# metaverse3d2022/Nerf-Cuda

Measured on AMD Instinct MI355X. Metric: megasamples/s (march samples composited into a ray = the reference's per-ray sample count), Lego-like NeRF render @1920x1080, higher is better.
Workload: dtype f16

## Files before the change

nerf-cuda_amd/csrc/nrf_device.h:

```cpp
#pragma once

#include <hip/hip_runtime.h>
#include <stdint.h>

#include "../../include/nerfhip.h"

namespace nrf {

typedef _Float16 half_t;
typedef _Float16 half2_t __attribute__((ext_vector_type(2)));
typedef _Float16 half4_t __attribute__((ext_vector_type(4)));
typedef _Float16 half8_t __attribute__((ext_vector_type(8)));
typedef float float2_t __attribute__((ext_vector_type(2)));
typedef float float4_t __attribute__((ext_vector_type(4)));

enum : uint32_t {
  LV_DENSE = 0,
  LV_HASH_POW2 = 1,
  LV_GENERIC = 2,
  LV_ADD_POW2 = 3
};

struct LevelParams {
  float scale;
// ... 287 lines not shown
  uint32_t log2H;
  float halfH;
  int log2_bound;
};

__device__ __forceinline__ MarchConst march_const(const DevModel& M, float dt_gamma) {
  MarchConst c;
  c.bound = M.bound;
  c.rbound = M.rbound;
  c.dt_gamma = dt_gamma;
  c.dt_min = 2 * 1.7320508075688772f / 1024;
  c.dt_max = 2 * M.bound / (float)M.H;
  c.H = M.H;
  c.C = M.cascade;
  c.HH = M.H * M.H;
  c.HHH = M.H * M.H * M.H;
  c.Hf = (float)M.H;
  c.Hm1 = (float)(M.H - 1);
  c.coarse_shift = M.coarse_shift;
  c.Hc = M.H >> M.coarse_shift;
  c.log2H = 31u - (uint32_t)__builtin_clz(M.H | 1u);
  c.halfH = 0.5f * (float)M.H;
  {
    int e;
    (void)frexpf(M.bound, &e);
    c.log2_bound = e - 1;
  }
  return c;
}

__device__ __forceinline__ float pcg32_first_float(uint64_t initstate, uint64_t initseq) {
  const uint64_t MULT = 0x5851f42d4c957f2dULL;
  const uint64_t inc = (initseq << 1u) | 1u;
  uint64_t state = inc;
  state += initstate;
  state = state * MULT + inc;
  const uint32_t xorshifted = (uint32_t)(((state >> 18u) ^ state) >> 27u);
  const uint32_t rot = (uint32_t)(state >> 59u);
  const uint32_t r = (xorshifted >> rot) | (xorshifted << ((~rot + 1u) & 31u));
  return __builtin_bit_cast(float, (r >> 9) | 0x3f800000u) - 1.0f;
}

enum : int { MARCH_FOUND = 0, MARCH_EXHAUSTED = 1, MARCH_OUT_OF_BUDGET = 2 };

__device__ __forceinline__ float clamp3(float x, float lo, float hi) { return __builtin_amdgcn_fmed3f(x, lo, hi); }

enum : int { MARCH_GENERIC = 0, MARCH_UNIT = 1, MARCH_POW2 = 2 };
template <bool COARSE, int MODE>
__device__ __forceinline__ int march_next(const MarchConst& c, const uint32_t* __restrict__ occ, const uint32_t* coarse,
                                          const float* ctab, float ox, float oy, float oz, float dx, float dy, float dz,
                                          float rdx, float rdy, float rdz, int sx, int sy, int sz, float far, float t_skip,
                                          int& budget, float& t, float& x, float& y, float& z, float& dt_out) {
  while (t < far) {
    if (budget <= 0) return MARCH_OUT_OF_BUDGET;
    --budget;
#ifdef NRF_DIAG_EXTRA_MARCH
#pragma unroll
    for (int e = 0; e < NRF_DIAG_EXTRA_MARCH; ++e) {
      float sink;
      asm volatile("v_mul_f32 %0, %1, %2" : "=v"(sink) : "v"(t), "v"(dx));
    }
#endif
#ifdef NRF_DIAG_FF_UPPER
    if (t < t_skip) {
      do {
        t += clamp3(t * c.dt_gamma, c.dt_min, c.dt_max);
      } while (t < t_skip && t < far);
      continue;
    }
#endif
    x = clamp3(ox + t * dx, -c.bound, c.bound);
    y = clamp3(oy + t * dy, -c.bound, c.bound);
    z = clamp3(oz + t * dz, -c.bound, c.bound);
    constexpr bool UNIT = MODE == MARCH_UNIT, POW2 = MODE == MARCH_POW2;
    int level = 0;
    int nx, ny, nz;
    if (UNIT) {
      nx = (int)clamp3(__builtin_fmaf(x, c.halfH, c.halfH), 0.0f, c.Hm1);
      ny = (int)clamp3(__builtin_fmaf(y, c.halfH, c.halfH), 0.0f, c.Hm1);
      nz = (int)clamp3(__builtin_fmaf(z, c.halfH, c.halfH), 0.0f, c.Hm1);
    } else if (POW2) {
      const float mx = fmaxf(fabsf(x), fmaxf(fabsf(y), fabsf(z)));
      int exponent;
      (void)frexpf(mx, &exponent);
      level = min(max(exponent, 0), (int)c.C - 1);
      const float scale = ldexpf(c.halfH, -min(level, c.log2_bound));
      nx = (int)clamp3(__builtin_fmaf(x, scale, c.halfH), 0.0f, c.Hm1);
      ny = (int)clamp3(__builtin_fmaf(y, scale, c.halfH), 0.0f, c.Hm1);
      nz = (int)clamp3(__builtin_fmaf(z, scale, c.halfH), 0.0f, c.Hm1);
    } else {
      float mip_bound = fminf(1.0f, c.bound), mip_rbound;
      if (c.C > 1) {
        const float mx = fmaxf(fabsf(x), fmaxf(fabsf(y), fabsf(z)));
        int exponent;
        (void)frexpf(mx, &exponent);
        level = (int)fminf((float)c.C - 1, fmaxf(0.0f, (float)exponent));
        mip_bound = fminf(ldexpf(1.0f, level), c.bound);
      }
      mip_rbound = (mip_bound == c.bound) ? c.rbound : ldexpf(1.0f, -level);
      nx = (int)clamp3((0.5f * (x * mip_rbound + 1)) * c.Hf, 0.0f, c.Hm1);
      ny = (int)clamp3((0.5f * (y * mip_rbound + 1)) * c.Hf, 0.0f, c.Hm1);
      nz = (int)clamp3((0.5f * (z * mip_rbound + 1)) * c.Hf, 0.0f, c.Hm1);
    }
    const uint32_t cell = (UNIT || POW2) ? ((((((uint32_t)level << c.log2H) | (uint32_t)nx) << c.log2H) | (uint32_t)ny) << c.log2H) | (uint32_t)nz
                                         : (uint32_t)level * c.HHH + (uint32_t)nx * c.HH + (uint32_t)ny * c.H + (uint32_t)nz;
    const float* tab = UNIT ? ctab : ctab + (uint32_t)level * (c.H + 1);
    const float bx = tab[nx + sx], by = tab[ny + sy], bz = tab[nz + sz];
    bool occupied = false;
    if (!(t < t_skip)) {
      if (COARSE) {
        const uint32_t lc = c.log2H - 2u;
        const uint32_t cc = (UNIT || POW2) ? (((((((uint32_t)level << lc) | ((uint32_t)nx >> 2)) << lc) | ((uint32_t)ny >> 2)) << lc) | ((uint32_t)nz >> 2))
                                           : ((uint32_t)level * c.Hc + ((uint32_t)nx >> 2)) * c.Hc * c.Hc + ((uint32_t)ny >> 2) * c.Hc + ((uint32_t)nz >> 2);
        const bool coarse_occ = (coarse[cc >> 5] >> (cc & 31u)) & 1u;
        if (coarse_occ) occupied = (occ[cell >> 5] >> (cell & 31u)) & 1u;
      } else {
        occupied = (occ[cell >> 5] >> (cell & 31u)) & 1u;
      }
    }
    if (occupied) {
      dt_out = clamp3(t * c.dt_gamma, c.dt_min, c.dt_max);
      return MARCH_FOUND;
    }
    const float tx = (bx - x) * rdx;
    const float ty = (by - y) * rdy;
    const float tz = (bz - z) * rdz;
    const float tt = t + fmaxf(0.0f, fminf(tx, fminf(ty, tz)));
    do {
      t += clamp3(t * c.dt_gamma, c.dt_min, c.dt_max);
    } while (t < tt);
  }
  return MARCH_EXHAUSTED;
}

#ifndef NRF_MARCH_FF
#define NRF_MARCH_FF 1
#endif
__device__ __forceinline__ float barrier_before(const float* ctab, int H, float mb, float mag, float o, float d, float rd, float t_skip) {
  const float NONE = -3.402823466e+38f;
  if (!(d < 0.0f) || !(rd > -3.0e38f)) return NONE;
  const float xs = o + t_skip * d;
  const float v = clamp3(ceilf((xs / mb + 1.0f) * (0.5f * (float)(H - 1))), 0.0f, (float)H);
  int n = (int)v;
  if (n > H - 1) return NONE;
  const float eps = 4.0e-6f * mag * (1.0f + fabsf(rd));
  float e = (ctab[n] - o) * rd + eps;
  if (!(e <= t_skip)) {
    if (++n > H - 1) return NONE;
    e = (ctab[n] - o) * rd + eps;
  }
  return e <= t_skip ? e : NONE;
}

__device__ __forceinline__ float fast_forward_to_barrier(const MarchConst& c, const float* ctab, float mb, const float o[3], const float d[3],
                                                         float rdx, float rdy, float rdz, float t, float t_skip, float far) {
  const float mag = t_skip + c.bound + 2.0f;
  const float tb = fminf(fmaxf(barrier_before(ctab, (int)c.H, mb, mag, o[0], d[0], rdx, t_skip),
                               fmaxf(barrier_before(ctab, (int)c.H, mb, mag, o[1], d[1], rdy, t_skip),
                                     barrier_before(ctab, (int)c.H, mb, mag, o[2], d[2], rdz, t_skip))), far);
  while (t < tb) t += clamp3(t * c.dt_gamma, c.dt_min, c.dt_max);
  return t;
}

__device__ __forceinline__ bool cube_interval(float s, const float o[3], const float rd[3], float& t_in, float& t_out) {
  bool ok = true;
  t_in = -3.402823466e+38f;
  t_out = 3.402823466e+38f;
#pragma unroll
  for (int a = 0; a < 3; ++a) {
    const float u = (-s - o[a]) * rd[a], v = (s - o[a]) * rd[a];
    ok = ok && (u == u) && (v == v);
    t_in = fmaxf(t_in, fminf(u, v));
    t_out = fminf(t_out, fmaxf(u, v));
  }
  return ok;
}

__device__ __forceinline__ float fast_forward_to_barrier_pow2(const MarchConst& c, const float* ctab, const float o[3], const float d[3],
                                                              float rdx, float rdy, float rdz, float t, float t_skip, float far) {
  const float NONE = -3.402823466e+38f;
  const float rd[3] = {rdx, rdy, rdz};
  const int C = (int)c.C, H = (int)c.H;
  const float mag = t_skip + c.bound + 2.0f;
  const float pad = 1.0e-4f * mag;
  const float slab0 = 2.0f / (float)H;
  float t_hi = t_skip, best = NONE;
  for (int it = 0; it <= C && !(best > NONE) && t_hi > t; ++it) {
    const float qx = clamp3(o[0] + t_hi * d[0], -c.bound, c.bound), qy = clamp3(o[1] + t_hi * d[1], -c.bound, c.bound),
                qz = clamp3(o[2] + t_hi * d[2], -c.bound, c.bound);
    int ex;
    (void)frexpf(fmaxf(fabsf(qx), fmaxf(fabsf(qy), fabsf(qz))), &ex);
    const int L = min(max(ex, 0), C - 1);
    const float mb = fminf(ldexpf(1.0f, L), c.bound);
    const float* tab = ctab + (uint32_t)L * (uint32_t)(H + 1);
    const float slab_next = slab0 * fminf(ldexpf(1.0f, L + 1), c.bound);
    const bool has_in = L >= 1, has_out = L <= C - 2;
    float ai = 0.f, bi = 0.f, ao = 0.f, bo = 0.f;
    const bool ok_in = has_in ? cube_interval(ldexpf(1.0f, L - 1) + pad, o, rd, ai, bi) : true;
    const bool ok_out = has_out ? cube_interval(ldexpf(1.0f, L) - pad, o, rd, ao, bo) : true;
#pragma unroll
    for (int a = 0; a < 3; ++a) {
      if (!(d[a] < 0.0f) || !(rd[a] > -3.0e38f)) continue;
      const float ard = fabsf(rd[a]);
      const float eps = 4.0e-6f * mag * (1.0f + ard);
      const float xs = o[a] + t_hi * d[a];
      int n = (int)clamp3(ceilf((xs / mb + 1.0f) * (0.5f * (float)(H - 1))), 0.0f, (float)H);
      if (n > H - 1) continue;
      float T = (tab[n] - o[a]) * rd[a], e = T + eps;
      if (!(e <= t_hi)) {
        if (++n > H - 1) continue;
        T = (tab[n] - o[a]) * rd[a];
        e = T + eps;
      }
      if (!(e <= t_hi)) continue;
      const float w_lo = T - slab_next * ard - eps;
      bool ok = ok_in && ok_out;
      if (has_out) ok = ok && ao <= w_lo && e <= bo;
      if (has_in) ok = ok && (ai > bi || e <= ai || w_lo >= bi);
      for (int Lp = L + 2; Lp <= C - 1 && ok; ++Lp) {
        float a2, b2;
        ok = cube_interval(ldexpf(1.0f, Lp - 1) - pad, o, rd, a2, b2);
        ok = ok && a2 <= T - slab0 * fminf(ldexpf(1.0f, Lp), c.bound) * ard - eps && e <= b2;
      }
      if (ok) best = fmaxf(best, e);
    }
    if (best > NONE) break;
    float nxt = NONE;
    const float lim = t_hi - 1.0e-6f * mag;
    if (has_in && ok_in) {
      if (ai < lim) nxt = fmaxf(nxt, ai);
      if (bi < lim) nxt = fmaxf(nxt, bi);
    }
    if (has_out && ok_out) {
      if (ao < lim) nxt = fmaxf(nxt, ao);
      if (bo < lim) nxt = fmaxf(nxt, bo);
    }
    t_hi = nxt - 4.0f * pad;
  }
  const float tb = fminf(best, far);
  while (t < tb) t += clamp3(t * c.dt_gamma, c.dt_min, c.dt_max);
  return t;
}

__device__ __forceinline__ half2_t weight_times_entry(float w, uint32_t entry) {
  float lo, hi;
  const float neg_zero = -0.0f;
  asm("v_fma_mix_f32 %0, %1, %2, %3 op_sel_hi:[0,1,0]" : "=v"(lo) : "v"(w), "v"(entry), "v"(neg_zero));
  asm("v_fma_mix_f32 %0, %1, %2, %3 op_sel:[0,1,0] op_sel_hi:[0,1,0]" : "=v"(hi) : "v"(w), "v"(entry), "v"(neg_zero));
  half2_t p;
  p.x = (half_t)lo;
  p.y = (half_t)hi;
  return p;
}

template <int UNI = 0, int SH = 2>
__device__ __forceinline__ void level_offsets(const LevelParams L, float px, float py, float pz, uint32_t (&off)[8], float (&frac)[3]) {
  float fx = px * L.scale; fx = fx + 0.5f;
  float fy = py * L.scale; fy = fy + 0.5f;
  float fz = pz * L.scale; fz = fz + 0.5f;
  const uint32_t gx = (uint32_t)(int)fx, gy = (uint32_t)(int)fy, gz = (uint32_t)(int)fz;
  frac[0] = __builtin_amdgcn_fractf(fx);
  frac[1] = __builtin_amdgcn_fractf(fy);
  frac[2] = __builtin_amdgcn_fractf(fz);

  const uint32_t level_off = L.off_b;
  {
    const bool hashed = UNI == 2 || (UNI == 0 && L.mode == LV_HASH_POW2);
    const uint32_t my = UNI == 2 ? (2654435761u << SH) : L.my_b;
    const uint32_t mz = UNI == 2 ? (805459861u << SH) : L.mz_b;
    const uint32_t mask = UNI == 1 ? 0xffffffffu : L.mask_b;
    const uint32_t ax0 = (gx << SH) + (hashed ? 0u : level_off);
    const uint32_t ax[2] = {ax0, ax0 + (1u << SH)};
    const uint32_t ay0 = gy * my, az0 = gz * mz;
    const uint32_t ay[2] = {ay0, ay0 + my};
    const uint32_t az[2] = {az0, az0 + mz};
    if (UNI == 2) {
      const uint32_t am[2] = {(ax[0] & mask) | level_off, (ax[1] & mask) | level_off};
      uint32_t bd[4];
#pragma unroll
      for (int q = 0; q < 4; ++q) bd[q] = (ay[q & 1] ^ az[q >> 1]) & mask;
#pragma unroll
      for (int c = 0; c < 8; ++c) off[c] = am[c & 1] ^ bd[c >> 1];
    } else if (UNI == 1) {
#pragma unroll
      for (int c = 0; c < 8; ++c) off[c] = ax[c & 1] + ay[(c >> 1) & 1] + az[(c >> 2) & 1];
    } else {
      const uint32_t axr[2] = {gx << SH, (gx << SH) + (1u << SH)};
      const uint32_t am[2] = {(axr[0] & mask) | level_off, (axr[1] & mask) | level_off};
#pragma unroll
      for (int q = 0; q < 4; ++q) {
        const uint32_t b = ay[q & 1], d = az[q >> 1];
        const uint32_t bd_x = (b ^ d) & mask, bd_s = b + d;
#pragma unroll
        for (int e = 0; e < 2; ++e) off[2 * q + e] = hashed ? (am[e] ^ bd_x) : (((axr[e] + bd_s) & mask) + level_off);
      }
    }
  }
}

template <int UNI = 0>
__device__ __forceinline__ void level_gather(const uint32_t* __restrict__ grid, uint32_t grid_bytes, const LevelParams L, float px,
                                             float py, float pz, uint32_t (&v)[8], float (&frac)[3]) {
  uint32_t off[8];
  level_offsets<UNI, 2>(L, px, py, pz, off, frac);
  const __amdgpu_buffer_rsrc_t rsrc = __builtin_amdgcn_make_buffer_rsrc(const_cast<uint32_t*>(grid), 0, grid_bytes, 0x00020000);
#ifdef NRF_DIAG_HASH_PAIRS
  if (UNI == 2) {
    typedef uint32_t u32x2 __attribute__((ext_vector_type(2)));
#pragma unroll
    for (int q = 0; q < 4; ++q) {
      const u32x2 w = __builtin_amdgcn_raw_buffer_load_b64(rsrc, off[2 * q] & ~4u, 0, 0);
      v[2 * q] = w.x;
      v[2 * q + 1] = w.y;
    }
    return;
  }
#endif
#pragma unroll
  for (int c = 0; c < 8; ++c) v[c] = __builtin_amdgcn_raw_buffer_load_b32(rsrc, off[c], 0, 0);
}

__device__ __forceinline__ void level_gather_quad(const uint32_t* __restrict__ grid, uint32_t grid_bytes, const LevelParams L, float px,
                                                  float py, float pz, uint32_t (&v)[8], float (&frac)[3]) {
  float fx = px * L.scale; fx = fx + 0.5f;
  float fy = py * L.scale; fy = fy + 0.5f;
  float fz = pz * L.scale; fz = fz + 0.5f;
  const uint32_t gx = (uint32_t)(int)fx, gy = (uint32_t)(int)fy, gz = (uint32_t)(int)fz;
  frac[0] = __builtin_amdgcn_fractf(fx);
  frac[1] = __builtin_amdgcn_fractf(fy);
  frac[2] = __builtin_amdgcn_fractf(fz);
  const uint32_t row = __umul24(gy, L.q_my_b) + L.q_off_b;
  const uint32_t slab = __umul24(gz, L.q_mz_b) + row;
  const uint32_t off0 = (gx << 4) + slab;
  const uint32_t off1 = off0 + L.q_mz_b;
  const __amdgpu_buffer_rsrc_t rsrc = __builtin_amdgcn_make_buffer_rsrc(const_cast<uint32_t*>(grid), 0, grid_bytes, 0x00020000);
  typedef uint32_t u32x4 __attribute__((ext_vector_type(4)));
  const u32x4 a = __builtin_amdgcn_raw_buffer_load_b128(rsrc, off0, 0, 0);
  const u32x4 b = __builtin_amdgcn_raw_buffer_load_b128(rsrc, off1, 0, 0);
  v[0] = a.x; v[1] = a.y; v[2] = a.z; v[3] = a.w;
  v[4] = b.x; v[5] = b.y; v[6] = b.z; v[7] = b.w;
}

__device__ __forceinline__ void level_gather_quad_far(const uint32_t* __restrict__ grid, const LevelParams L, float px, float py, float pz,
                                                      uint32_t (&v)[8], float (&frac)[3]) {
  float fx = px * L.scale; fx = fx + 0.5f;
  float fy = py * L.scale; fy = fy + 0.5f;
  float fz = pz * L.scale; fz = fz + 0.5f;
  uint32_t gx = (uint32_t)(int)fx, gy = (uint32_t)(int)fy, gz = (uint32_t)(int)fz;
  frac[0] = __builtin_amdgcn_fractf(fx);
  frac[1] = __builtin_amdgcn_fractf(fy);
  frac[2] = __builtin_amdgcn_fractf(fz);
  gx = gx < L.q_max ? gx : L.q_max;
  gy = gy < L.q_max ? gy : L.q_max;
  gz = gz < L.q_max ? gz : L.q_max;
  const uint32_t row = __umul24(gy, L.q_my_b) + L.q_off_b;
  const uint32_t cell = __umul24(gz, L.q_mz_b) + row + gx;
  const uint4* q = reinterpret_cast<const uint4*>(grid) + cell;
  const uint4 a = q[0];
  const uint4 b = q[L.q_mz_b];
  v[0] = a.x; v[1] = a.y; v[2] = a.z; v[3] = a.w;
  v[4] = b.x; v[5] = b.y; v[6] = b.z; v[7] = b.w;
}

template <bool FAST = false>
__device__ __forceinline__ uint32_t level_interp(const uint32_t (&v)[8], const float (&frac)[3]) {
  const float wx[2] = {1 - frac[0], frac[0]};
  const float wy[2] = {1 - frac[1], frac[1]};
  const float wz[2] = {1 - frac[2], frac[2]};
  if constexpr (FAST) {
    uint32_t a = 0u;
#pragma unroll
    for (int c = 0; c < 8; ++c) {
      const float w = (wx[c & 1] * wy[(c >> 1) & 1]) * wz[(c >> 2) & 1];
      asm("v_fma_mixlo_f16 %0, %1, %2, %0 op_sel_hi:[0,1,1]" : "+v"(a) : "v"(w), "v"(v[c]));
      asm("v_fma_mixhi_f16 %0, %1, %2, %0 op_sel:[0,1,1] op_sel_hi:[0,1,1]" : "+v"(a) : "v"(w), "v"(v[c]));
    }
    return a;
  }
  half2_t acc = {(half_t)0.0f, (half_t)0.0f};
#ifdef NRF_DIAG_DROP_INTERP_CVT
  float diag_acc_lo = 0.f, diag_acc_hi = 0.f;
#endif
#pragma unroll
  for (int c = 0; c < 8; ++c) {
    const float w = (wx[c & 1] * wy[(c >> 1) & 1]) * wz[(c >> 2) & 1];
#ifdef NRF_DIAG_DROP_INTERP_CVT
    {
      float lo, hi;
      const float neg_zero = -0.0f;
      asm("v_fma_mix_f32 %0, %1, %2, %3 op_sel_hi:[0,1,0]" : "=v"(lo) : "v"(w), "v"(v[c]), "v"(neg_zero));
      asm("v_fma_mix_f32 %0, %1, %2, %3 op_sel:[0,1,0] op_sel_hi:[0,1,0]" : "=v"(hi) : "v"(w), "v"(v[c]), "v"(neg_zero));
      diag_acc_lo += lo;
      diag_acc_hi += hi;
    }
// ... 482 lines not shown
```

nerf-cuda_amd/csrc/nrf_render.h:

```cpp

#pragma once
#include <cstddef>
#include <cstdlib>

#include "nrf_device.h"
#include "nrf_generic.h"
#include "nrf_launch.h"

namespace nrf {

#ifndef NRF_SLOTS
#define NRF_SLOTS 64
#endif
constexpr int SLOTS = NRF_SLOTS;
struct WaveLds {
  union {
    float4 pos[SLOTS];
    float4 out[SLOTS];
  };
  float2 aux[SLOTS];
  uint32_t dirf[64][8];
};
static_assert(sizeof(WaveLds) == 2048 + 24 * SLOTS, "WaveLds layout");

// ... 988 lines not shown
        }
        if (!(c_in < c_out)) continue;
        float t_last, t_first;
        const uint32_t* dl_g = M.occ_dilated + (size_t)k * M.dilated_level_words;
        const uint32_t* dl_l = dil_lds + (size_t)k * M.dilated_level_words;
        const bool vis = use_dil_lds ? coarse_visibility(dl_l, Hc, mb, o, d, rdx, rdy, rdz, c_in, c_out, t_first, t_last)
                                     : coarse_visibility(dl_g, Hc, mb, o, d, rdx, rdy, rdz, c_in, c_out, t_first, t_last);
        if (vis) {
          any = true;
          first = fminf(first, t_first);
          last = fmaxf(last, t_last);
        }
      }
      alive = any;
      if (last < far_m) far_m = last;
      if (any) t_skip = first;
#if NRF_MARCH_FF
      if (any && P.march_ff != 0) {
        const float* tab = COARSE_LDS ? ctab_lds : M.cell_bound;
        if (MARCH == MARCH_UNIT) t = fast_forward_to_barrier(mc, tab, 1.0f, o, d, rdx, rdy, rdz, t, t_skip, far_m);
        else if (MARCH == MARCH_POW2 || mc.C > 1) t = fast_forward_to_barrier_pow2(mc, tab, o, d, rdx, rdy, rdz, t, t_skip, far_m);
        else t = fast_forward_to_barrier(mc, tab, fminf(1.0f, mc.bound), o, d, rdx, rdy, rdz, t, t_skip, far_m);
      }
#endif
    }
    if (RAYS != RAYS_DENSITY && alive) {
      float u0 = 0.5f * d[0]; u0 = u0 + 0.5f;
      float u1 = 0.5f * d[1]; u1 = u1 + 0.5f;
      float u2 = 0.5f * d[2]; u2 = u2 + 0.5f;
      if constexpr (GEN) {
        lm.gen.rayd[3 * lane] = u0;
        lm.gen.rayd[3 * lane + 1] = u1;
        lm.gen.rayd[3 * lane + 2] = u2;
      } else {
        half_t e[16];
        encode_dir16(M, u0, u1, u2, e);
#pragma unroll
        for (int j = 0; j < 8; ++j) {
          half2_t h;
          h.x = e[2 * j];
          h.y = e[2 * j + 1];
          W->dirf[lane][j] = h2_bits(h);
        }
        if constexpr (NET == NET_WIDE) {
          lm.gen.rayd[3 * lane] = u0;
          lm.gen.rayd[3 * lane + 1] = u1;
          lm.gen.rayd[3 * lane + 2] = u2;
        }
      }
    }
    if (__syncthreads_or(alive ? 1 : 0) != 0) {
      if constexpr (!GEN) {
        stage_fragments<NET>(M, wl);
        __syncthreads();
      }
    }
  }
  if (!valid_tile) return;
  NRF_STAMP(t_setup_done);
  TileAcc acc;
  TileStats ts;
  const uint32_t pix_idx = P.tile_major ? (uint32_t)k_local * 64u + (uint32_t)lane : (uint32_t)py * (uint32_t)P.W + (uint32_t)px;
  tile_rounds<NET, COARSE_LDS, MARCH, false, false, PERTURB, RAYS>(M, P, mc, lm, coarse_lds, ctab_lds, lane, o, d, rdx, rdy, rdz, sx, sy, sz,
                                                                   far_m, t_skip, t, tc, alive, acc, ts, 0, nullptr, pix_idx, 0.f, 0.f, nullptr,
                                                                   view);
  const unsigned n_samples = ts.n_samples, n_rounds = ts.n_rounds, n_tile_slots = ts.n_tile_slots;
  const unsigned n_composited = ts.n_composited;
#ifdef NRF_PHASE_TIMING
  const unsigned long long c_march = ts.c_march, c_net = ts.c_net, c_comp = ts.c_comp;
  const unsigned n_lane_trips = ts.n_lane_trips, n_wave_iters = ts.n_wave_iters;
#endif

  {
    const uint32_t rn = (uint32_t)py * (uint32_t)P.W + (uint32_t)px;
    float dn;
    const float4 c = finish_pixel<RAYS != RAYS_NONE>(P, acc, near, far, view, rn, in_img && rn < P.rays_per_view, dn);
    store_pixel(P, rgba, depth, k_local, lane, px, py, in_img, c, dn);
  }
  counters += (blockIdx.x % COUNTER_SLOTS) * 16;
  if (lane == 0 && n_rounds != 0) {
    atomicAdd(&counters[0], (unsigned long long)n_samples);
    atomicAdd(&counters[1], (unsigned long long)n_rounds);
    atomicAdd(&counters[11], (unsigned long long)n_tile_slots);
    atomicAdd(&counters[7], (unsigned long long)n_composited);
  }
#ifdef NRF_PHASE_TIMING
  if (lane == 0) {
    NRF_STAMP(t_end);
    atomicMin(&wg_first, t_begin);
    atomicMax(&wg_last, t_end);
    __threadfence_block();
    const unsigned valid_waves = min((unsigned)RENDER_WAVES, (unsigned)(P.n_local_tiles - (k_local - wave)));
    if (atomicAdd(&wg_done, 1u) + 1u == valid_waves) {
      atomicAdd(&counters[12], (unsigned long long)valid_waves * (wg_last - wg_first));
      atomicAdd(&counters[13], 1ull);
    }
    atomicAdd(&counters[2], c_march);
    atomicAdd(&counters[3], c_net);
    atomicAdd(&counters[4], c_comp);
    atomicAdd(&counters[5], t_end - t_begin);
    atomicAdd(&counters[6], 1ull);
    atomicAdd(&counters[9], (unsigned long long)n_wave_iters);
    atomicAdd(&counters[10], t_setup_done - t_begin);
  }
#endif
#ifdef NRF_PHASE_TIMING
  {
    unsigned lt = n_lane_trips;
    for (int o = 32; o; o >>= 1) lt += __shfl_xor(lt, o);
    if (lane == 0) atomicAdd(&counters[8], (unsigned long long)lt);
  }
#endif
}

template <int NET>
__device__ __forceinline__ void encode_ray_dir(const DevModel& M, const LdsMap& lm, int lane, const float (&d)[3]) {
  float u0 = 0.5f * d[0]; u0 = u0 + 0.5f;
  float u1 = 0.5f * d[1]; u1 = u1 + 0.5f;
  float u2 = 0.5f * d[2]; u2 = u2 + 0.5f;
  if constexpr (NET == NET_GENERIC) {
    lm.gen.rayd[3 * lane] = u0;
    lm.gen.rayd[3 * lane + 1] = u1;
    lm.gen.rayd[3 * lane + 2] = u2;
  } else if constexpr (NET == NET_WIDE_SH) {
    half_t* row = lm.gen.dir + (size_t)lane * SH_ROW_HALVES;
    gen_encode_dir(M, *M.gen, u0, u1, u2, row);
    const uint32_t* r32 = reinterpret_cast<const uint32_t*>(row);
#pragma unroll
    for (int j = 0; j < 8; ++j) lm.W->dirf[lane][j] = r32[j];
  } else {
    half_t e[16];
    encode_dir16(M, u0, u1, u2, e);
#pragma unroll
    for (int j = 0; j < 8; ++j) {
      half2_t h;
      h.x = e[2 * j];
      h.y = e[2 * j + 1];
      lm.W->dirf[lane][j] = h2_bits(h);
    }
    if constexpr (NET == NET_WIDE) {
      lm.gen.rayd[3 * lane] = u0;
      lm.gen.rayd[3 * lane + 1] = u1;
      lm.gen.rayd[3 * lane + 2] = u2;
    }
  }
}

__host__ __device__ constexpr int persist_waves(int net) {
  return net == NET_WIDE_SH ? 8 : ((net == NET_GENERIC || net == NET_WIDE || net == NET_W128 || net == NET_ACT) ? 12 : 16);
}
constexpr int LDS_CLOCK_BYTES = 16;
constexpr int LDS_QUEUE_BYTES = (MAX_VIEWS + 2) * 4 + 80 + LDS_CLOCK_BYTES;
static_assert(sizeof(HelpLds) + LDS_CLOCK_BYTES <= 80 + LDS_CLOCK_BYTES, "HelpLds and the clock stamps live behind the scheduler word");

struct PersistArgs {
  DevModel M;
  FrameParams P;
  ViewBatch VB;
};
static_assert(offsetof(PersistArgs, P) == (sizeof(DevModel) + alignof(FrameParams) - 1) / alignof(FrameParams) * alignof(FrameParams) &&
                  offsetof(PersistArgs, VB) % alignof(ViewBatch) == 0,
              "PersistArgs mirrors the kernarg segment of render_persistent_kernel");

template <int NET, int MARCH, int WAVES = persist_waves(NET), bool WLDS = false, bool U8 = false, int RAYS = RAYS_NONE,
          uint32_t GP = GATHER_RUNTIME, bool FAST = false>
__global__ __launch_bounds__(64 * WAVES, 1) void render_persistent_kernel(const DevModel M0, const FrameParams P0, const ViewBatch VB0,
                                                                              float4* __restrict__ rgba0, float* __restrict__ depth0,
                                                                              unsigned long long* __restrict__ counters,
                                                                              unsigned* __restrict__ queue) {
  extern __shared__ __attribute__((aligned(16))) unsigned char smem[];
  const int wave = __builtin_amdgcn_readfirstlane((int)(threadIdx.x >> 6));
  const int lane = lane_id();
  typedef const PersistArgs __attribute__((address_space(4))) * KArgPtr;
  KArgPtr ka = (KArgPtr)__builtin_amdgcn_kernarg_segment_ptr();
  const DevModel& M = M0;
  const FrameParams& P = P0;
  const ViewBatch& VB = VB0;
  constexpr int PERSIST_WAVES = WAVES;
  constexpr bool GEN = NET == NET_GENERIC;
  constexpr int OUT8 = U8 ? 1 : 0;
  LdsMap lm = lds_map<NET>(smem, M, wave, PERSIST_WAVES);
  uint32_t* coarse_lds = reinterpret_cast<uint32_t*>(lm.tables);
  float* ctab_lds = reinterpret_cast<float*>(coarse_lds + M.lds_coarse_words);
  uint32_t* dil_lds = reinterpret_cast<uint32_t*>(ctab_lds + M.lds_ctab_floats);
  int* q_lds = reinterpret_cast<int*>(dil_lds + M.lds_dilated_words);
  unsigned* sched = reinterpret_cast<unsigned*>(q_lds + MAX_VIEWS + 1);
  HelpLds* hl = reinterpret_cast<HelpLds*>(sched + 1);
  static_assert(WAVES <= 16, "HelpLds::mail / idle_mask hold 16 waves");
  if constexpr (!GEN) stage_fragments<NET>(M, lm.wl);
  if constexpr (GEN && WLDS) {
    uint4* w_lds = reinterpret_cast<uint4*>(smem + ((reinterpret_cast<unsigned char*>(hl + 1) + LDS_CLOCK_BYTES - smem + 15) & ~(size_t)15));
    for (uint32_t i = threadIdx.x; i < M.gen_frag_bytes / 16u; i += blockDim.x) w_lds[i] = M.wfrag[i];
    lm.gen.wfrag = w_lds;
  }
  for (uint32_t i = threadIdx.x; i < M.lds_coarse_words; i += blockDim.x) coarse_lds[i] = M.occ_coarse[i];
  for (uint32_t i = threadIdx.x; i < M.lds_ctab_floats; i += blockDim.x) ctab_lds[i] = M.cell_bound[i];
  for (uint32_t i = threadIdx.x; i < M.lds_dilated_words; i += blockDim.x) dil_lds[i] = M.occ_dilated[i];
  if constexpr (plan_levels(GP)) {
    if (threadIdx.x < 16) stage_plan_level<GP>(lm.lvs, threadIdx.x, M.lv[threadIdx.x]);
  } else {
    if (threadIdx.x < 16) lm.lvs[threadIdx.x] = M.lv[threadIdx.x];
  }
  if (threadIdx.x <= MAX_VIEWS) {
    const int v = (int)threadIdx.x;
    q_lds[v] = v < VB.n_views ? VB.v[v].q_begin : VB.q_total;
  }
  if (threadIdx.x == 0) *sched = (0xfffffeu << 5) | 4u;
  if (threadIdx.x == 0) {
    hl->idle_mask = 0u;
    hl->busy = PERSIST_WAVES;
  }
  if (threadIdx.x < 16) hl->mail[threadIdx.x] = 0u;
  __syncthreads();
#ifndef NRF_PHASE_TIMING
  unsigned* clk_lds = reinterpret_cast<unsigned*>(hl + 1);
  if (wave == 0) {
    unsigned long long t0, r0;
    asm volatile("s_memtime %0\n\ts_memrealtime %1\n\ts_waitcnt lgkmcnt(0)" : "=s"(t0), "=s"(r0)::"memory");
    if (lane == 0) {
      clk_lds[0] = (unsigned)t0;
      clk_lds[1] = (unsigned)(t0 >> 32);
      clk_lds[2] = (unsigned)r0;
      clk_lds[3] = (unsigned)(r0 >> 32);
    }
  }
#endif

  const MarchConst mc = march_const(M, P.dt_gamma);
  TileStats ts;
  const unsigned n_cls = (unsigned)VB0.n_classes, cls_cols = (unsigned)VB0.class_cols, n_units = (unsigned)VB0.q_total;
  const unsigned cls0 = (__builtin_amdgcn_s_getreg(20 | (0 << 6) | (3 << 11)) & 15u) % n_cls;
  constexpr unsigned POS_DONE = 0xffffffu;
  NRF_STAMP(t_loop_begin);
#ifdef NRF_PHASE_TIMING
  unsigned long long c_sched = 0;
  const unsigned long long t_rt_begin = stamp_rt();
#endif
  while (true) {
    NRF_STAMP(t_sched0);
    unsigned pos, bt, moved;
    while (true) {
      unsigned old = 0u;
      if (lane == 0) old = atomicAdd(sched, 1u);
      old = (unsigned)__builtin_amdgcn_readfirstlane((int)old);
      moved = old >> 29;
      pos = (old >> 5) & POS_DONE;
      bt = old & 31u;
      if (pos == POS_DONE || bt < 4u) break;
      if (bt == 4u) {
        unsigned nb = POS_DONE;
        for (; moved < n_cls; ++moved) {
          const unsigned cls = (cls0 + moved) % n_cls;
          const unsigned total = n_units * ((cls_cols - cls + n_cls - 1u) / n_cls);
          unsigned got = 0u;
          if (lane == 0) got = atomicAdd(queue + cls, 1u);
          got = (unsigned)__builtin_amdgcn_readfirstlane((int)got);
          if (got < total) { nb = got; break; }
        }
        if (nb == POS_DONE) moved = 0u;
        else if (P0.plan_order != nullptr) {
          unsigned off = 0u;
          const unsigned cls = (cls0 + moved) % n_cls;
          for (unsigned c2 = 0; c2 < cls; ++c2) off += n_units * ((cls_cols - c2 + n_cls - 1u) / n_cls);
          nb = P0.plan_order[off + nb];
        }
        if (lane == 0) __hip_atomic_store(sched, (moved << 29) | (nb << 5) | 1u, __ATOMIC_RELEASE, __HIP_MEMORY_SCOPE_WORKGROUP);
        pos = nb;
        bt = 0u;
        break;
      }
      while ((__hip_atomic_load(sched, __ATOMIC_ACQUIRE, __HIP_MEMORY_SCOPE_WORKGROUP) >> 5) == (old >> 5)) __builtin_amdgcn_s_sleep(2);
    }
    NRF_STAMP(t_sched1);
    NRF_ACC(c_sched, t_sched0, t_sched1);
    if (pos == POS_DONE) break;
    asm volatile("" : "+s"(ka));
    const DevModel& M = *(const DevModel*)&ka->M;
    const FrameParams& P = *(const FrameParams*)&ka->P;
    const ViewBatch& VB = *(const ViewBatch*)&ka->VB;
    const unsigned cls = (cls0 + moved) % n_cls, ncols = (cls_cols - cls + n_cls - 1u) / n_cls;
    const int u = (int)(pos / ncols), j = (int)(pos - (unsigned)u * ncols);
    static_assert(MAX_VIEWS == 128, "two ballots cover the views");
    const int view = __popcll(__ballot(lane < VB.n_views && u >= q_lds[lane])) +
                     __popcll(__ballot(lane + 64 < VB.n_views && u >= q_lds[lane + 64])) - 1;
    const ViewParams& V = VB.v[view];
    const int ul = u - V.q_begin;
    const bool co = P.centre_out != 0;
    auto centre_out = [co](int i, int n) { const int off = (i + 1) >> 1; return co ? (n - 1) / 2 + ((i & 1) ? off : -off) : i; };
    const int sxn = (P.tiles_x + 3) >> 2, N = P.shard_count;
    const int row = V.q_row0 + centre_out(ul, V.q_rows);
    const int s_row = row * sxn;
    const int ls_first = s_row > P.shard_index ? (s_row - P.shard_index + N - 1) / N : 0;
    const int ls = ls_first + (int)cls + (int)n_cls * j;
    if (ls * N + P.shard_index >= s_row + sxn) continue;
    const int k_local = ls * 4 + (int)bt;
    if (k_local >= V.k_hi || k_local >= P.n_local_tiles) continue;
    const OutPlanes op = view_planes<OUT8>(P, rgba0, depth0, view, VB.view_stride_px);
    float4* rgba = op.rgba;
    float* depth = op.depth;
    const int strips_x = (P.tiles_x + 3) >> 2;
    const int strip = (k_local >> 2) * P.shard_count + P.shard_index;
    const int tx = (strip % strips_x) * 4 + (k_local & 3), ty = strip / strips_x;
    const int px = tx * 8 + (lane & 7), py = ty * 8 + (lane >> 3);
    const bool in_img = px < P.W && py < P.H;
    const float4 background = make_float4(P.bg_color, P.bg_color, P.bg_color, 0.f);
    if (tx * 8 > V.roi[2] || tx * 8 + 7 < V.roi[0] || ty * 8 > V.roi[3] || ty * 8 + 7 < V.roi[1]) {
      store_pixel<OUT8, true>(P, rgba, depth, k_local, lane, px, py, in_img, background, 0.f);
      if constexpr (U8) if (tx < P.tiles_x) tile_written(P, view, ty, lane);
      continue;
    }
    NRF_STAMP(t_begin);
#ifdef NRF_PHASE_TIMING
    const unsigned samples_before = ts.n_samples;
#endif
    float o[3] = {V.org[0], V.org[1], V.org[2]};
    float d[3];
    bool has_ray = true;
    if constexpr (RAYS != RAYS_NONE) has_ray = load_ray(P, view, (uint32_t)py * (uint32_t)P.W + (uint32_t)px, in_img, o, d);
    else ray_dir(V.R, V.cam, px, py, d);
    float near, far;
    near_far(M.aabb, o, d, P.min_near, near, far);
    if constexpr (RAYS != RAYS_NONE) {
      if (!has_ray) near = far = 3.402823466e+38f;
      else clamp_ray(P, view, (uint32_t)py * (uint32_t)P.W + (uint32_t)px, near, far);
    }
    const float rdx = 1 / d[0], rdy = 1 / d[1], rdz = 1 / d[2];
    const int sx = __builtin_signbitf(d[0]) ? 0 : 1;
    const int sy = __builtin_signbitf(d[1]) ? 0 : 1;
    const int sz = __builtin_signbitf(d[2]) ? 0 : 1;
    float t = near, tc = near;
    bool alive = in_img && (near < far);
    float far_m = far, t_skip = near, t_in, t_out;
    box_interval(M.occ_box, o, rdx, rdy, rdz, t_in, t_out);
    const bool nan = !(t_in == t_in) || !(t_out == t_out);
    {
      const bool hits = (M.occ_box[0] <= M.occ_box[3]) && (t_in <= t_out) && (t_out > near);
      if (t_out < far_m) far_m = t_out;
      if (nan) far_m = far;
      alive = alive && (hits || nan);
    }
    if (M.occ_dilated != nullptr && alive && !nan) {
      const int Hc = (int)(M.H >> 2);
      const float t_box0 = fmaxf(t_in, near);
      bool any = false;
      float first = far_m, last = t_box0;
      const uint32_t n_casc = MARCH == MARCH_UNIT ? 1u : M.cascade;
      for (uint32_t k = 0; k < n_casc; ++k) {
        const float mb = (n_casc > 1) ? fminf(ldexpf(1.0f, (int)k), M.bound) : fminf(1.0f, M.bound);
        float c_in = t_box0, c_out = far_m;
        if (n_casc > 1) {
          const float cube[6] = {-mb, -mb, -mb, mb, mb, mb};
          float a, b;
          box_interval(cube, o, rdx, rdy, rdz, a, b);
          if (a == a && b == b) {
            c_in = fmaxf(c_in, a);
            c_out = fminf(c_out, b);
          }
        }
        if (!(c_in < c_out)) continue;
        float t_last, t_first;
        if (coarse_visibility(dil_lds + (size_t)k * M.dilated_level_words, Hc, mb, o, d, rdx, rdy, rdz, c_in, c_out, t_first, t_last)) {
          any = true;
          first = fminf(first, t_first);
          last = fmaxf(last, t_last);
        }
      }
      alive = any;
      if (last < far_m) far_m = last;
      if (any) t_skip = first;
#if NRF_MARCH_FF
      if (any && P.march_ff != 0) {
        if (MARCH == MARCH_UNIT) t = fast_forward_to_barrier(mc, ctab_lds, 1.0f, o, d, rdx, rdy, rdz, t, t_skip, far_m);
        else if (MARCH == MARCH_POW2 || mc.C > 1) t = fast_forward_to_barrier_pow2(mc, ctab_lds, o, d, rdx, rdy, rdz, t, t_skip, far_m);
        else t = fast_forward_to_barrier(mc, ctab_lds, fminf(1.0f, mc.bound), o, d, rdx, rdy, rdz, t, t_skip, far_m);
      }
#endif
    }
    TileAcc acc;
    bool given = false;
    const uint32_t pix_idx = P.tile_major ? (uint32_t)k_local * 64u + (uint32_t)lane : (uint32_t)py * (uint32_t)P.W + (uint32_t)px;
    if (__ballot(alive) != 0ull) {
      if (RAYS != RAYS_DENSITY && alive) encode_ray_dir<NET>(M, lm, lane, d);
      wave_sync();
      NRF_STAMP(t_setup_done);
      const HelpArgs ha = {hl, lm.W - wave, view};
      tile_rounds<NET, true, MARCH, true, FAST, false, RAYS, GP>(M, P, mc, lm, coarse_lds, ctab_lds, lane, o, d, rdx, rdy, rdz, sx, sy, sz, far_m, t_skip,
                                                             t, tc, alive, acc, ts, 0, &ha, pix_idx, near, far, &given,
                                                             view);
#ifdef NRF_PHASE_TIMING
      if (lane == 0) {
        NRF_STAMP(t_end);
        atomicAdd(&counters[(blockIdx.x % COUNTER_SLOTS) * 16 + 5], t_end - t_begin);
        atomicAdd(&counters[(blockIdx.x % COUNTER_SLOTS) * 16 + 6], 1ull);
        atomicAdd(&counters[(blockIdx.x % COUNTER_SLOTS) * 16 + 10], t_setup_done - t_begin);
      }
#endif
    }
    float dn;
    const uint32_t rn = (uint32_t)py * (uint32_t)P.W + (uint32_t)px;
    const float4 c = finish_pixel<RAYS != RAYS_NONE>(P, acc, near, far, view, rn, in_img && rn < P.rays_per_view, dn);
#ifdef NRF_PHASE_TIMING
    if (P.march_budget == 4095) {
      NRF_STAMP(t_tile_end);
      const unsigned hw_id = __builtin_amdgcn_s_getreg((4 << 0) | (0 << 6) | (31 << 11));
      dn = (lane & 7) == 1 ? (float)(t_tile_end - t_begin) * 1e-6f
         : (lane & 7) == 2 ? (float)(ts.n_samples - samples_before) * 1e-3f
         : (lane & 7) == 3 ? (float)bt
         : (lane & 7) == 4 ? (float)((hw_id >> 4) & 3u)
         : (lane & 7) == 5 ? (float)wave
         : (lane & 7) == 6 ? (float)(hw_id & 15u)
         : (float)(t_begin - t_loop_begin) * 1e-6f;
    }
#endif
    const unsigned long long given_mask = __ballot(given);
    if (given_mask == 0ull) {
      store_pixel<OUT8>(P, rgba, depth, k_local, lane, px, py, in_img, c, dn);
    } else if (!given && (in_img || P.tile_major)) {
      const bool pad = !in_img;
      store_ray_pixel<OUT8>(P, rgba, depth, pix_idx, pad ? make_float4(0.f, 0.f, 0.f, 0.f) : c, pad ? 0.f : dn);
    }
    if constexpr (U8) if (tx < P.tiles_x) tile_written(P, view, ty, lane, 64u - (unsigned)__popcll(given_mask));
  }
// ... 222 lines not shown
```

Before: 15480.

## Prefetch next work strip into LDS park slot and unroll barrier fast-forward stepping

The persistent kernel's scheduler now keeps a parked next-strip word in LDS. The wave that exhausts the current strip publishes the already-fetched next strip immediately and then fetches the following one, which takes the global queue atomic and plan_order lookup off the critical path of the waves waiting on it. The scheme adds a two-stage boot protocol and a spin on the park word, so it is more complex and carries more risk of ordering mistakes. Separately, the fast-forward loop to the occupancy barrier now evaluates three steps per iteration before checking, which cuts loop-carried branch overhead.

```diff
diff --git a/nerf-cuda_amd/csrc/nrf_device.h b/nerf-cuda_amd/csrc/nrf_device.h
--- a/nerf-cuda_amd/csrc/nrf_device.h
+++ b/nerf-cuda_amd/csrc/nrf_device.h
@@ -463,14 +463,30 @@
   return e <= t_skip ? e : NONE;
 }
 
+#ifndef NRF_FF_STEP4
+#define NRF_FF_STEP4 1
+#endif
+__device__ __forceinline__ float step_to_barrier(const MarchConst& c, float t, float tb) {
+#if NRF_FF_STEP4
+  while (true) {
+    const float t1 = t + clamp3(t * c.dt_gamma, c.dt_min, c.dt_max);
+    const float t2 = t1 + clamp3(t1 * c.dt_gamma, c.dt_min, c.dt_max);
+    const float t3 = t2 + clamp3(t2 * c.dt_gamma, c.dt_min, c.dt_max);
+    if (!(t3 < tb)) break;
+    t = t3 + clamp3(t3 * c.dt_gamma, c.dt_min, c.dt_max);
+  }
+#endif
+  while (t < tb) t += clamp3(t * c.dt_gamma, c.dt_min, c.dt_max);
+  return t;
+}
+
 __device__ __forceinline__ float fast_forward_to_barrier(const MarchConst& c, const float* ctab, float mb, const float o[3], const float d[3],
                                                          float rdx, float rdy, float rdz, float t, float t_skip, float far) {
   const float mag = t_skip + c.bound + 2.0f;
   const float tb = fminf(fmaxf(barrier_before(ctab, (int)c.H, mb, mag, o[0], d[0], rdx, t_skip),
                                fmaxf(barrier_before(ctab, (int)c.H, mb, mag, o[1], d[1], rdy, t_skip),
                                      barrier_before(ctab, (int)c.H, mb, mag, o[2], d[2], rdz, t_skip))), far);
-  while (t < tb) t += clamp3(t * c.dt_gamma, c.dt_min, c.dt_max);
-  return t;
+  return step_to_barrier(c, t, tb);
 }
 
 __device__ __forceinline__ bool cube_interval(float s, const float o[3], const float rd[3], float& t_in, float& t_out) {
@@ -548,9 +564,7 @@
     }
     t_hi = nxt - 4.0f * pad;
   }
-  const float tb = fminf(best, far);
-  while (t < tb) t += clamp3(t * c.dt_gamma, c.dt_min, c.dt_max);
-  return t;
+  return step_to_barrier(c, t, fminf(best, far));
 }
 
 __device__ __forceinline__ half2_t weight_times_entry(float w, uint32_t entry) {
diff --git a/nerf-cuda_amd/csrc/nrf_render.h b/nerf-cuda_amd/csrc/nrf_render.h
--- a/nerf-cuda_amd/csrc/nrf_render.h
+++ b/nerf-cuda_amd/csrc/nrf_render.h
@@ -1164,6 +1164,11 @@
 constexpr int LDS_CLOCK_BYTES = 16;
 constexpr int LDS_QUEUE_BYTES = (MAX_VIEWS + 2) * 4 + 80 + LDS_CLOCK_BYTES;
 static_assert(sizeof(HelpLds) + LDS_CLOCK_BYTES <= 80 + LDS_CLOCK_BYTES, "HelpLds and the clock stamps live behind the scheduler word");
+#ifndef NRF_SCHED_PREFETCH
+#define NRF_SCHED_PREFETCH 1
+#endif
+constexpr int LDS_PARK_BYTES = NRF_SCHED_PREFETCH ? 4 : 0;
+static_assert(sizeof(HelpLds) + LDS_CLOCK_BYTES + LDS_PARK_BYTES <= 80 + LDS_CLOCK_BYTES, "the parked strip's word lies behind the clock stamps");
 
 struct PersistArgs {
   DevModel M;
@@ -1217,7 +1222,18 @@
     const int v = (int)threadIdx.x;
     q_lds[v] = v < VB.n_views ? VB.v[v].q_begin : VB.q_total;
   }
-  if (threadIdx.x == 0) *sched = (0xfffffeu << 5) | 4u;
+  constexpr bool PREFETCH = NRF_SCHED_PREFETCH != 0 && GP != GATHER_RUNTIME;
+  static_assert(!(PREFETCH && GEN), "the generic instance's staged fragments begin behind the clock stamps, where `park` lies");
+  unsigned* park = reinterpret_cast<unsigned*>(hl + 1) + LDS_CLOCK_BYTES / 4;
+  constexpr unsigned POS_BOOT = 0xfffffeu, POS_BOOT2 = 0xfffffdu, PARK_PENDING = 0xffffffffu;
+  if constexpr (PREFETCH) {
+    if (threadIdx.x == 0) {
+      *sched = (POS_BOOT << 5) | 3u;
+      *park = PARK_PENDING;
+    }
+  } else {
+    if (threadIdx.x == 0) *sched = (0xfffffeu << 5) | 4u;
+  }
   if (threadIdx.x == 0) {
     hl->idle_mask = 0u;
     hl->busy = PERSIST_WAVES;
@@ -1258,28 +1274,72 @@
       moved = old >> 29;
       pos = (old >> 5) & POS_DONE;
       bt = old & 31u;
-      if (pos == POS_DONE || bt < 4u) break;
-      if (bt == 4u) {
-        unsigned nb = POS_DONE;
-        for (; moved < n_cls; ++moved) {
-          const unsigned cls = (cls0 + moved) % n_cls;
-          const unsigned total = n_units * ((cls_cols - cls + n_cls - 1u) / n_cls);
-          unsigned got = 0u;
-          if (lane == 0) got = atomicAdd(queue + cls, 1u);
-          got = (unsigned)__builtin_amdgcn_readfirstlane((int)got);
-          if (got < total) { nb = got; break; }
+      if constexpr (PREFETCH) {
+        if (pos == POS_DONE || bt < 3u) break;
+        if (bt == 3u) {
+          const bool first = pos == POS_BOOT, boot = pos >= POS_BOOT2;
+          unsigned m = 0u;
+          bool more = true;
+          if (!first) {
+            unsigned e;
+            while ((e = __hip_atomic_load(park, __ATOMIC_ACQUIRE, __HIP_MEMORY_SCOPE_WORKGROUP)) == PARK_PENDING) __builtin_amdgcn_s_sleep(1);
+            e = (unsigned)__builtin_amdgcn_readfirstlane((int)e);
+            unsigned pending = PARK_PENDING;
+            asm volatile("" : "+s"(pending));
+            if (lane == 0) {
+              __hip_atomic_store(park, pending, __ATOMIC_RELAXED, __HIP_MEMORY_SCOPE_WORKGROUP);
+              __hip_atomic_store(sched, e, __ATOMIC_RELEASE, __HIP_MEMORY_SCOPE_WORKGROUP);
+            }
+            m = e >> 29;
+            more = ((e >> 5) & POS_DONE) != POS_DONE;
+          }
+          if (more) {
+            unsigned nb = POS_DONE;
+            for (; m < n_cls; ++m) {
+              const unsigned cls = (cls0 + m) % n_cls;
+              const unsigned total = n_units * ((cls_cols - cls + n_cls - 1u) / n_cls);
+              unsigned got = 0u;
+              if (lane == 0) got = atomicAdd(queue + cls, 1u);
+              got = (unsigned)__builtin_amdgcn_readfirstlane((int)got);
+              if (got < total) { nb = got; break; }
+            }
+            if (nb == POS_DONE) m = 0u;
+            else if (P0.plan_order != nullptr) {
+              unsigned off = 0u;
+              const unsigned cls = (cls0 + m) % n_cls;
+              for (unsigned c2 = 0; c2 < cls; ++c2) off += n_units * ((cls_cols - c2 + n_cls - 1u) / n_cls);
+              nb = P0.plan_order[off + nb];
+            }
+            if (lane == 0) __hip_atomic_store(park, (m << 29) | (nb << 5), __ATOMIC_RELEASE, __HIP_MEMORY_SCOPE_WORKGROUP);
+          }
+          if (first && lane == 0) __hip_atomic_store(sched, (POS_BOOT2 << 5) | 3u, __ATOMIC_RELEASE, __HIP_MEMORY_SCOPE_WORKGROUP);
+          if (boot) continue;
+          break;
         }
-        if (nb == POS_DONE) moved = 0u;
-        else if (P0.plan_order != nullptr) {
-          unsigned off = 0u;
-          const unsigned cls = (cls0 + moved) % n_cls;
-          for (unsigned c2 = 0; c2 < cls; ++c2) off += n_units * ((cls_cols - c2 + n_cls - 1u) / n_cls);
-          nb = P0.plan_order[off + nb];
+      } else {
+        if (pos == POS_DONE || bt < 4u) break;
+        if (bt == 4u) {
+          unsigned nb = POS_DONE;
+          for (; moved < n_cls; ++moved) {
+            const unsigned cls = (cls0 + moved) % n_cls;
+            const unsigned total = n_units * ((cls_cols - cls + n_cls - 1u) / n_cls);
+            unsigned got = 0u;
+            if (lane == 0) got = atomicAdd(queue + cls, 1u);
+            got = (unsigned)__builtin_amdgcn_readfirstlane((int)got);
+            if (got < total) { nb = got; break; }
+          }
+          if (nb == POS_DONE) moved = 0u;
+          else if (P0.plan_order != nullptr) {
+            unsigned off = 0u;
+            const unsigned cls = (cls0 + moved) % n_cls;
+            for (unsigned c2 = 0; c2 < cls; ++c2) off += n_units * ((cls_cols - c2 + n_cls - 1u) / n_cls);
+            nb = P0.plan_order[off + nb];
+          }
+          if (lane == 0) __hip_atomic_store(sched, (moved << 29) | (nb << 5) | 1u, __ATOMIC_RELEASE, __HIP_MEMORY_SCOPE_WORKGROUP);
+          pos = nb;
+          bt = 0u;
+          break;
         }
-        if (lane == 0) __hip_atomic_store(sched, (moved << 29) | (nb << 5) | 1u, __ATOMIC_RELEASE, __HIP_MEMORY_SCOPE_WORKGROUP);
-        pos = nb;
-        bt = 0u;
-        break;
       }
       while ((__hip_atomic_load(sched, __ATOMIC_ACQUIRE, __HIP_MEMORY_SCOPE_WORKGROUP) >> 5) == (old >> 5)) __builtin_amdgcn_s_sleep(2);
     }
```

Measured after the change: 15420. No clear change (-0.3%).
